# thu-ml/stochastic_gcn

Hardware: AMD Instinct MI355X
Metric: training edges/s (SpMM) (higher is better)
Workload: dtype f32

## Files before the change

### stochastic_gcn_amd/csrc/sgcn_csplan.cpp

```cpp
#include "sgcn_host.h"
#include "../../include/sgcn.h"

#include <algorithm>
#include <atomic>
#include <climits>
#include <cmath>
#include <cstdint>
#include <cstdio>
#include <cstdlib>
#include <cstring>
#include <functional>
#include <memory>
#include <new>
#include <numeric>
#include <queue>
#include <thread>
#include <vector>

#include <sched.h>

namespace {

struct VRow { int32_t row, piece, npieces, nnz; };

int plan_threads(int32_t requested) {
    if (requested > 0) return std::min<int32_t>(requested, 256);
    if (const char* e = getenv("SGCN_PLAN_THREADS")) {
        const int v = atoi(e);
        if (v > 0) return std::min(v, 256);
    }
    int n = (int)std::thread::hardware_concurrency();
    cpu_set_t set;
    if (sched_getaffinity(0, sizeof(set), &set) == 0) n = CPU_COUNT(&set);
    if (FILE* f = fopen("/sys/fs/cgroup/cpu.max", "r")) {
        char q[64] = {0};
        long long period = 0;
        if (fscanf(f, "%63s %lld", q, &period) == 2 && strcmp(q, "max") != 0 && period > 0) {
            const long long quota = atoll(q);
            if (quota > 0) n = (int)std::min<long long>(n, std::max<long long>(1, quota / period));
        }
        fclose(f);
    }
    return std::max(1, std::min(n, 64));
}

template <class F>
bool run_threads(int nthr, F fn) {
    std::atomic<int> bad{0};
    auto guarded = [&](int tid) {
        try { fn(tid); } catch (...) { bad.store(1); }
    };
    if (nthr <= 1) { guarded(0); return !bad.load(); }
    std::vector<std::thread> pool;
    pool.reserve((size_t)nthr - 1);
    try {
        for (int t = 1; t < nthr; t++) pool.emplace_back(guarded, t);
    } catch (...) { bad.store(1); }
    guarded(0);
    for (auto& th : pool) th.join();
    return !bad.load();
}

template <class F>
bool parallel_chunks(int64_t n, int64_t chunk, int nthr, F fn) {
    if (n <= 0) return true;
    chunk = std::max<int64_t>(1, chunk);
    nthr = (int)std::max<int64_t>(1, std::min<int64_t>(nthr, (n + chunk - 1) / chunk));
    std::atomic<int64_t> next{0};
    return run_threads(nthr, [&](int tid) {
        for (;;) {
            const int64_t b = next.fetch_add(chunk);
            if (b >= n) break;
            fn(b, std::min(n, b + chunk), tid);
        }
    });
}

void bucket_rows(const int32_t* row_group, int32_t M, std::vector<int32_t>& order, std::vector<int64_t>& gptr) {
    order.resize((size_t)M);
    if (!row_group) {
        std::iota(order.begin(), order.end(), 0);
        gptr = {0, (int64_t)M};
        return;
    }
    int32_t ng = 0;
    for (int32_t r = 0; r < M; r++) ng = std::max(ng, row_group[r] + 1);
    gptr.assign((size_t)ng + 1, 0);
    for (int32_t r = 0; r < M; r++) gptr[(size_t)row_group[r] + 1]++;
    for (int32_t g = 0; g < ng; g++) gptr[(size_t)g + 1] += gptr[g];
    std::vector<int64_t> fill(gptr.begin(), gptr.end() - 1);
    for (int32_t r = 0; r < M; r++) order[(size_t)fill[row_group[r]]++] = r;
}

inline int32_t default_t(const int32_t* rowptr, int32_t M) {
    const int64_t avg = M > 0 ? ((int64_t)rowptr[M] - rowptr[0]) / M : 0;
    return (int32_t)std::min<int64_t>(1024, std::max<int64_t>(64, 8 * avg));
}

void make_vrows(const int32_t* rowptr, const int32_t* rows, int64_t nrows, int32_t T, std::vector<VRow>& v) {
    std::vector<VRow> tmp;
    tmp.reserve((size_t)nrows + 64);
    int32_t wmax = 0;
    for (int64_t ri = 0; ri < nrows; ri++) {
        const int32_t r = rows[ri];
        const int32_t n = rowptr[r + 1] - rowptr[r];
        if (n <= T) { tmp.push_back({r, 0, 1, n}); wmax = std::max(wmax, n); continue; }
        const int32_t c = (n + T - 1) / T;
        for (int32_t q = 0; q < c; q++) {
            const int32_t w = (n - q + c - 1) / c;
            tmp.push_back({r, q, c, w});
            wmax = std::max(wmax, w);
        }
    }
    std::vector<int64_t> start((size_t)wmax + 2, 0);
    for (const VRow& x : tmp) start[(size_t)(wmax - x.nnz) + 1]++;
    for (size_t i = 1; i < start.size(); i++) start[i] += start[i - 1];
    const size_t base = v.size();
    v.resize(base + tmp.size());
    for (const VRow& x : tmp) v[base + (size_t)start[(size_t)(wmax - x.nnz)]++] = x;
}

void deal(const VRow* v, int64_t nv, int64_t vbase, int32_t R, int64_t nbins, int64_t* assign) {
    std::fill(assign, assign + nbins * R, (int64_t)-1);
    std::vector<int32_t> fill((size_t)nbins, 0);
    typedef std::pair<int64_t, int64_t> WT;
    std::priority_queue<WT, std::vector<WT>, std::greater<WT>> heap;
    for (int64_t t = 0; t < nbins; t++) heap.push({0, t});
    for (int64_t i = 0; i < nv; i++) {
        WT top = heap.top();
        heap.pop();
        const int64_t t = top.second;
        assign[t * R + fill[t]++] = vbase + i;
        if (fill[t] < R) heap.push({top.first + v[i].nnz, t});
    }
}

struct Layout {
    int32_t R = 16;
    int32_t NG = 1;
    std::vector<VRow> v;
    std::vector<int64_t> assign;
    int64_t ntiles = 0;
};

void layout_g1(const int32_t* rowptr, int32_t M, int32_t R, int32_t T, const int32_t* row_group, Layout& L) {
    std::vector<int32_t> order;
    std::vector<int64_t> gptr;
    bucket_rows(row_group, M, order, gptr);
    L.R = R; L.NG = 1; L.ntiles = 0;
    std::vector<int64_t> first_tile, vbase;
    for (size_t g = 0; g + 1 < gptr.size(); g++) {
        vbase.push_back((int64_t)L.v.size());
        make_vrows(rowptr, order.data() + gptr[g], gptr[g + 1] - gptr[g], T, L.v);
        first_tile.push_back(L.ntiles);
        L.ntiles += ((int64_t)L.v.size() - vbase.back() + R - 1) / R;
    }
    L.assign.resize((size_t)L.ntiles * R);
    for (size_t g = 0; g + 1 < gptr.size(); g++) {
        const int64_t nv = (g + 2 < gptr.size() ? vbase[g + 1] : (int64_t)L.v.size()) - vbase[g];
        const int64_t nt = (nv + R - 1) / R;
        deal(L.v.data() + vbase[g], nv, vbase[g], R, nt, L.assign.data() + first_tile[g] * R);
    }
}

constexpr int kG2R = 16;
void layout_gn(const int32_t* rowptr, int32_t M, int32_t T, int32_t round_tiles, int NG, Layout& L) {
    std::vector<int32_t> rows((size_t)M);
    std::iota(rows.begin(), rows.end(), 0);
    make_vrows(rowptr, rows.data(), M, T, L.v);
    const int64_t nv = (int64_t)L.v.size();
    int64_t nt = (nv + NG * kG2R - 1) / (NG * kG2R);
    if (round_tiles > 0 && nt > round_tiles / 2)
        nt = (nt + round_tiles - 1) / round_tiles * round_tiles;
    L.R = kG2R; L.NG = NG; L.ntiles = nt;
    L.assign.resize((size_t)nt * NG * kG2R);
    deal(L.v.data(), nv, 0, kG2R, nt * NG, L.assign.data());
}

struct Csr {
    const int32_t* rowptr = nullptr;
    const int32_t* col = nullptr;
    const float* val = nullptr;
    std::vector<int32_t> own_col;
    std::vector<float> own_val;
};

int prepare_csr(const int32_t* rowptr, const int32_t* col, const float* val, int32_t M, int bits, int nthr, Csr& A) {
    A.rowptr = rowptr; A.col = col; A.val = val;
    std::atomic<int> unsorted{0}, bad{0};
    const int64_t lim = (int64_t)1 << bits;
    if (!parallel_chunks(M, 2048, nthr, [&](int64_t r0, int64_t r1, int) {
            int u = 0, b = 0;
            for (int64_t r = r0; r < r1; r++)
                for (int32_t p = rowptr[r]; p < rowptr[r + 1]; p++) {
                    b |= (col[p] < 0) | ((int64_t)col[p] >= lim);
                    if (p > rowptr[r]) u |= col[p] < col[p - 1];
                }
            if (u) unsorted.store(1);
            if (b) bad.store(1);
        })) return 2;
    if (bad.load()) return 1;
    if (!unsorted.load()) return 0;
    const int64_t nnz = (int64_t)rowptr[M] - rowptr[0];
    const int64_t p0 = rowptr[0];
    try {
        A.own_col.resize((size_t)nnz);
        if (val) A.own_val.resize((size_t)nnz);
    } catch (...) { return 2; }
    if (!parallel_chunks(M, 512, nthr, [&](int64_t r0, int64_t r1, int) {
            std::vector<std::pair<int32_t, float>> buf;
            for (int64_t r = r0; r < r1; r++) {
                buf.clear();
                for (int32_t p = rowptr[r]; p < rowptr[r + 1]; p++) buf.push_back({col[p], val ? val[p] : 0.f});
                std::stable_sort(buf.begin(), buf.end(),
                                 [](const std::pair<int32_t, float>& a, const std::pair<int32_t, float>& b) { return a.first < b.first; });
                for (size_t i = 0; i < buf.size(); i++) {
                    A.own_col[(size_t)(rowptr[r] - p0) + i] = buf[i].first;
                    if (val) A.own_val[(size_t)(rowptr[r] - p0) + i] = buf[i].second;
                }
            }
        })) return 2;
    A.col = A.own_col.data() - p0;
    if (val) A.val = A.own_val.data() - p0;
    return 0;
}

struct Ent { uint32_t col, pos; float val; uint32_t lr; };
struct Scratch { std::vector<Ent> a, b; std::vector<uint32_t> runs, runs2; };

const std::vector<Ent>& gather_bin(const Layout& L, const Csr& A, int64_t bin, const uint32_t* warp, int32_t wshift, Scratch& S) {
    S.a.clear();
    S.runs.clear();
    S.runs.push_back(0);
    for (int32_t k = 0; k < L.R; k++) {
        const int64_t vi = L.assign[(size_t)bin * L.R + k];
        if (vi < 0) continue;
        const VRow& vr = L.v[(size_t)vi];
        const int32_t b = A.rowptr[vr.row], e = A.rowptr[vr.row + 1];
        for (int32_t p = b + vr.piece; p < e; p += vr.npieces) {
            const uint32_t c = (uint32_t)A.col[p];
            S.a.push_back({c, warp ? warp[c >> wshift] : c, A.val ? A.val[p] : 0.f, (uint32_t)k});
        }
        if (S.a.size() > S.runs.back()) S.runs.push_back((uint32_t)S.a.size());
    }
    std::vector<Ent>* src = &S.a;
    std::vector<Ent>* dst = &S.b;
    std::vector<uint32_t>* rs = &S.runs;
    std::vector<uint32_t>* rd = &S.runs2;
    while (rs->size() > 2) {
        dst->resize(src->size());
        rd->clear();
        rd->push_back(0);
        const size_t nr = rs->size() - 1;
        for (size_t i = 0; i < nr; i += 2) {
            const uint32_t lo = (*rs)[i], mid = (*rs)[i + 1], hi = i + 1 < nr ? (*rs)[i + 2] : mid;
            const Ent* x = src->data() + lo;
            const Ent* xe = src->data() + mid;
            const Ent* y = xe;
            const Ent* ye = src->data() + hi;
// ... 17 lines not shown
    int64_t step = 0;
    uint32_t window = 0;
    for (;;) {
        int64_t lo = INT64_MAX;
        uint32_t lo_col = 0;
        for (int g = 0; g < NG; g++)
            if (pos[g] < e[g]->size() && (int64_t)(*e[g])[pos[g]].pos < lo) { lo = (*e[g])[pos[g]].pos; lo_col = (*e[g])[pos[g]].col; }
        if (lo == INT64_MAX) break;
        window = lo_col;
        for (int g = 0; g < NG; g++) {
            const bool has = pos[g] < e[g]->size();
            const bool take = has && (align <= 0 || (int64_t)(*e[g])[pos[g]].pos <= lo + align);
            emit(g, take ? &(*e[g])[pos[g]] : nullptr, window);
            pos[g] += take;
        }
        step++;
    }
    const int64_t per_chunk = 64 / NG;
    while (step % per_chunk != 0) {
        for (int g = 0; g < NG; g++) emit(g, nullptr, window);
        step++;
    }
    return step;
}

inline uint64_t pack_entry(uint32_t word, float v) {
    uint32_t bits;
    memcpy(&bits, &v, 4);
    return (uint64_t)word | ((uint64_t)bits << 32);
}

}

struct sgcn_csbuild {
    int32_t G = 1, R = 16, T = 0;
    int64_t ntiles = 0, nentries = 0, nfix = 0, nslots = 0;
    bool count_only = false;
    std::vector<int64_t> tile_ptr;
    std::vector<int32_t> tile_rows, tile_slots;
    std::vector<sgcn_fix_t> fix;
    std::unique_ptr<uint64_t[]> flat;
    std::vector<std::vector<uint64_t>> arena;
    std::vector<int32_t> tile_tid;
    std::vector<int64_t> tile_off;
    int nthreads = 1;
};

namespace {

int build_plan(const int32_t* rowptr, const int32_t* col, const float* val, int32_t M, int32_t G, int32_t R, int32_t T,
               int32_t round_tiles, int32_t align, const int32_t* row_group, const uint32_t* warp, int32_t wshift,
               int32_t nthreads, bool count_only, sgcn_csbuild* B) {
    const int nthr = plan_threads(nthreads);
    B->G = G; B->R = G == 1 ? R : kG2R; B->nthreads = nthr; B->count_only = count_only;
    if (T <= 0) T = default_t(rowptr, M);
    B->T = T;
    if (row_group)
        for (int32_t r = 0; r < M; r++)
            if (row_group[r] < 0) return sgcn::fail(SGCN_ERR_INVALID, "csplan_build: negative group label at row %d", r);
    std::vector<int32_t> first_slot((size_t)M, -1);
    {
        int64_t slot = 0;
        for (int32_t r = 0; r < M; r++) {
            const int64_t n = (int64_t)rowptr[r + 1] - rowptr[r];
            if (n < 0) return sgcn::fail(SGCN_ERR_INVALID, "csplan_build: rowptr not monotone at %d", r);
            if (n <= T) continue;
            const int32_t c = (int32_t)((n + T - 1) / T);
            first_slot[r] = (int32_t)slot;
            B->fix.push_back(sgcn_fix_t{r, (int32_t)slot, c});
            slot += c;
            if (slot > INT32_MAX) return sgcn::fail(SGCN_ERR_INVALID, "csplan_build: too many workspace slots");
        }
        B->nfix = (int64_t)B->fix.size();
        B->nslots = slot;
    }
    const int bits = (G == 1 && R > 16) ? 27 : 28;
    Csr A;
    if (M > 0) {
        const int rc = prepare_csr(rowptr, col, val, M, bits, nthr, A);
        if (rc == 1) return sgcn::fail(SGCN_ERR_INVALID, "csplan_build: a column does not fit %d bits", bits);
        if (rc == 2) return sgcn::fail(SGCN_ERR_INVALID, "csplan_build: out of host memory");
    }
    Layout L;
    if (G == 1) layout_g1(rowptr, M, R, T, row_group, L);
    else layout_gn(rowptr, M, T, round_tiles, G, L);
    const int64_t nt = L.ntiles;
    const int32_t RR = L.R * L.NG;
    B->ntiles = nt;
    B->tile_ptr.assign((size_t)nt + 1, 0);
    B->tile_rows.resize((size_t)nt * RR);
    B->tile_slots.resize((size_t)nt * RR);
    auto fill_rows = [&](int64_t t) {
        for (int32_t k = 0; k < RR; k++) {
            const int64_t s = t * RR + k;
            const int64_t vi = L.assign[(size_t)s];
            if (vi < 0) { B->tile_rows[(size_t)s] = -1; B->tile_slots[(size_t)s] = -1; continue; }
            const VRow& vr = L.v[(size_t)vi];
            B->tile_rows[(size_t)s] = vr.row;
            B->tile_slots[(size_t)s] = vr.npieces > 1 ? first_slot[vr.row] + vr.piece : -1;
        }
    };
    const uint32_t shift = (uint32_t)bits;
    if (G == 1) {
        for (int64_t t = 0; t < nt; t++) {
            int64_t n = 0;
            for (int32_t k = 0; k < RR; k++) {
                const int64_t vi = L.assign[(size_t)(t * RR + k)];
                if (vi >= 0) n += L.v[(size_t)vi].nnz;
            }
            B->tile_ptr[(size_t)t + 1] = B->tile_ptr[(size_t)t] + n;
        }
        B->nentries = B->tile_ptr[(size_t)nt];
        if (count_only) { for (int64_t t = 0; t < nt; t++) fill_rows(t); return SGCN_OK; }
        B->flat.reset(new (std::nothrow) uint64_t[(size_t)std::max<int64_t>(B->nentries, 1)]);
        if (!B->flat) return sgcn::fail(SGCN_ERR_INVALID, "csplan_build: out of host memory");
        uint64_t* flat = B->flat.get();
        const bool ok = parallel_chunks(nt, 8, nthr, [&](int64_t t0, int64_t t1, int) {
            Scratch S;
            for (int64_t t = t0; t < t1; t++) {
                fill_rows(t);
                const std::vector<Ent>& e = gather_bin(L, A, t, nullptr, 0, S);
                uint64_t* o = flat + B->tile_ptr[(size_t)t];
                for (const Ent& en : e) *o++ = pack_entry(en.col | (en.lr << shift), en.val);
            }
        });
        if (!ok) return sgcn::fail(SGCN_ERR_INVALID, "csplan_build: out of host memory");
        return SGCN_OK;
    }
    B->arena.resize((size_t)nthr);
    B->tile_tid.assign((size_t)nt, 0);
    B->tile_off.assign((size_t)nt, 0);
    std::vector<int64_t> tile_len((size_t)nt, 0);
    const int64_t nnz = M > 0 ? (int64_t)rowptr[M] - rowptr[0] : 0;
    const int NG = G;
    const bool ok = parallel_chunks(nt, 8, nthr, [&](int64_t t0, int64_t t1, int tid) {
        Scratch S[4];
        const std::vector<Ent>* e[4] = {nullptr, nullptr, nullptr, nullptr};
        std::vector<uint64_t>& ar = B->arena[(size_t)tid];
        if (!count_only && ar.capacity() == 0) ar.reserve((size_t)(nnz / nthr + nnz / (4 * nthr) + 4096));
        for (int64_t t = t0; t < t1; t++) {
            fill_rows(t);
            for (int g = 0; g < NG; g++) e[g] = &gather_bin(L, A, NG * t + g, warp, wshift, S[g]);
            B->tile_tid[(size_t)t] = tid;
            B->tile_off[(size_t)t] = (int64_t)ar.size();
            int64_t steps;
            if (count_only) {
                steps = gn_schedule(e, NG, align, [](int, const Ent*, uint32_t) {});
            } else {
                steps = gn_schedule(e, NG, align, [&](int, const Ent* en, uint32_t window) {
                    if (en) {
                        float v = en->val;
                        uint32_t bts;
                        memcpy(&bts, &v, 4);
                        if (bts == kPadBits) v = 0.0f;
                        ar.push_back(pack_entry(en->col | (en->lr << 28), v));
                    } else {
                        ar.push_back((uint64_t)window | ((uint64_t)kPadBits << 32));
                    }
                });
            }
            tile_len[(size_t)t] = steps * NG;
        }
    });
    if (!ok) return sgcn::fail(SGCN_ERR_INVALID, "csplan_build: out of host memory");
    for (int64_t t = 0; t < nt; t++) B->tile_ptr[(size_t)t + 1] = B->tile_ptr[(size_t)t] + tile_len[(size_t)t];
    B->nentries = B->tile_ptr[(size_t)nt];
    return SGCN_OK;
}

int export_plan(const sgcn_csbuild* B, int64_t* tile_ptr, int32_t* colrow, float* valout, int32_t* tile_rows,
                int32_t* tile_slots, sgcn_fix_t* fix) {
    if (B->count_only) return sgcn::fail(SGCN_ERR_INVALID, "csbuild_export: a count-only build holds no entries");
    if (B->ntiles > 0 && (!tile_ptr || !tile_rows || !tile_slots)) return sgcn::fail(SGCN_ERR_INVALID, "csbuild_export: bad argument");
    if (B->nentries > 0 && (!colrow || !valout)) return sgcn::fail(SGCN_ERR_INVALID, "csbuild_export: bad argument");
    if (B->nfix > 0 && !fix) return sgcn::fail(SGCN_ERR_INVALID, "csbuild_export: split rows but no fix array");
    if (tile_ptr) memcpy(tile_ptr, B->tile_ptr.data(), B->tile_ptr.size() * sizeof(int64_t));
    if (B->tile_rows.size()) {
        memcpy(tile_rows, B->tile_rows.data(), B->tile_rows.size() * sizeof(int32_t));
        memcpy(tile_slots, B->tile_slots.data(), B->tile_slots.size() * sizeof(int32_t));
    }
    if (B->nfix) memcpy(fix, B->fix.data(), B->fix.size() * sizeof(sgcn_fix_t));
    auto split = [&](const uint64_t* src, int64_t n, int64_t at) {
        for (int64_t i = 0; i < n; i++) {
            colrow[at + i] = (int32_t)(uint32_t)src[i];
            const uint32_t bits = (uint32_t)(src[i] >> 32);
            memcpy(valout + at + i, &bits, 4);
        }
    };
    if (B->G == 1) {
        parallel_chunks(B->nentries, 1 << 18, B->nthreads, [&](int64_t b, int64_t e, int) { split(B->flat.get() + b, e - b, b); });
        return SGCN_OK;
    }
    parallel_chunks(B->ntiles, 8, B->nthreads, [&](int64_t t0, int64_t t1, int) {
        for (int64_t t = t0; t < t1; t++)
            split(B->arena[(size_t)B->tile_tid[(size_t)t]].data() + B->tile_off[(size_t)t],
                  B->tile_ptr[(size_t)t + 1] - B->tile_ptr[(size_t)t], B->tile_ptr[(size_t)t]);
    });
    return SGCN_OK;
}

}

extern "C" {

int sgcn_csplan_build(const int32_t* rowptr, const int32_t* col, const float* val, int32_t M, int32_t ngroups, int32_t R,
                      int32_t T, int32_t round_tiles, int32_t align, const int32_t* row_group, const uint32_t* host_warp,
                      int32_t warp_shift, int32_t nthreads, sgcn_csbuild_t** out) {
    if (!out) return sgcn::fail(SGCN_ERR_INVALID, "csplan_build: bad argument");
    *out = nullptr;
    if (M < 0 || (M > 0 && (!rowptr || !col || !val))) return sgcn::fail(SGCN_ERR_INVALID, "csplan_build: bad argument");
    if (ngroups != 1 && ngroups != 2 && ngroups != 4) return sgcn::fail(SGCN_ERR_INVALID, "csplan_build: one, two or four lane groups per wavefront");
    if (ngroups == 1 && (R < 1 || R > 32)) return sgcn::fail(SGCN_ERR_INVALID, "csplan_build: 1 <= R <= 32");
    if (ngroups != 1 && row_group) return sgcn::fail(SGCN_ERR_INVALID, "csplan_build: plans with lane groups are ungrouped");
    if (host_warp && (warp_shift < 0 || warp_shift > 27)) return sgcn::fail(SGCN_ERR_INVALID, "csplan_build: bad warp_shift");
    sgcn_csbuild* B = new (std::nothrow) sgcn_csbuild();
    if (!B) return sgcn::fail(SGCN_ERR_INVALID, "csplan_build: out of host memory");
    int rc;
    try {
        rc = build_plan(rowptr, col, val, M, ngroups, R, T, round_tiles, align, row_group, host_warp, warp_shift, nthreads, false, B);
    } catch (...) {
        rc = sgcn::fail(SGCN_ERR_INVALID, "csplan_build: out of host memory");
    }
    if (rc != SGCN_OK) { delete B; return rc; }
    *out = B;
    return SGCN_OK;
}

int sgcn_csbuild_sizes(const sgcn_csbuild_t* b, int64_t* ntiles, int64_t* nentries, int64_t* nfix, int64_t* nslots,
                       int32_t* T_used, int32_t* threads_used) {
    if (!b) return sgcn::fail(SGCN_ERR_INVALID, "csbuild_sizes: bad argument");
    if (ntiles) *ntiles = b->ntiles;
    if (nentries) *nentries = b->nentries;
    if (nfix) *nfix = b->nfix;
    if (nslots) *nslots = b->nslots;
    if (T_used) *T_used = b->T;
    if (threads_used) *threads_used = b->nthreads;
    return SGCN_OK;
}

int sgcn_csbuild_export(const sgcn_csbuild_t* b, int64_t* tile_ptr, int32_t* colrow, float* valout, int32_t* tile_rows,
                        int32_t* tile_slots, sgcn_fix_t* fix) {
    if (!b) return sgcn::fail(SGCN_ERR_INVALID, "csbuild_export: bad argument");
    return export_plan(b, tile_ptr, colrow, valout, tile_rows, tile_slots, fix);
}

void sgcn_csbuild_free(sgcn_csbuild_t* b) { delete b; }

// ... 244 lines not shown
```

### stochastic_gcn_amd/csrc/sgcn_spmm.hip

```cpp
#include "sgcn_dev.h"
#include <cstring>

namespace sgcn {

namespace {
int g_tune_nv = 0;
int g_tune_unroll = 0;
int g_tune_slabmajor = 1;
int g_tune_cs_round = 0;
int g_tune_cs_unroll = 0;
int g_tune_cs_pace = 0;
int g_tune_cs_slack = 0;
int g_tune_cs_noextra = 0;
int g_tune_step_overlap = 1;
int g_tune_step_fuse = 127;
int g_tune_cs_g2_wide = 0;
int g_tune_cs_nowarp = 0;
int g_tune_cs_last_pct = 80;
int g_tune_gemm_min_steps = 0;
int g_tune_gemm_mb16_slice_k = 0;
int g_tune_lds_wave_bias = 100;
int g_tune_lds_mix = 1;
int g_tune_lds_dbg = 0;
thread_local int tl_step_overlap = -1, tl_step_fuse = -1;
}

void step_mode_override(int overlap, int fuse) { tl_step_overlap = overlap; tl_step_fuse = fuse; }

int tune_get(const char* key) {
    if (!strcmp(key, "spmm_nv")) return g_tune_nv;
    if (!strcmp(key, "spmm_unroll")) return g_tune_unroll;
    if (!strcmp(key, "spmm_slabmajor")) return g_tune_slabmajor;
    if (!strcmp(key, "cs_round")) return g_tune_cs_round;
    if (!strcmp(key, "cs_unroll")) return g_tune_cs_unroll;
    if (!strcmp(key, "cs_pace")) return g_tune_cs_pace;
    if (!strcmp(key, "cs_slack")) return g_tune_cs_slack;
    if (!strcmp(key, "cs_noextra")) return g_tune_cs_noextra;
    if (!strcmp(key, "step_overlap")) return tl_step_overlap >= 0 ? tl_step_overlap : g_tune_step_overlap;
    if (!strcmp(key, "step_fuse")) return tl_step_fuse >= 0 ? tl_step_fuse : g_tune_step_fuse;
    if (!strcmp(key, "cs_g2_wide")) return g_tune_cs_g2_wide;
    if (!strcmp(key, "cs_nowarp")) return g_tune_cs_nowarp;
    if (!strcmp(key, "cs_last_pct")) return g_tune_cs_last_pct;
    if (!strcmp(key, "gemm_min_steps")) return g_tune_gemm_min_steps;
    if (!strcmp(key, "gemm_mb16_slice_k")) return g_tune_gemm_mb16_slice_k;
    if (!strcmp(key, "lds_wave_bias")) return g_tune_lds_wave_bias;
    if (!strcmp(key, "lds_mix")) return g_tune_lds_mix;
    if (!strcmp(key, "lds_dbg")) return g_tune_lds_dbg;
    return -1;
}

struct SpmmArgs {
    const int32_t* rowptr;
    const int32_t* col;
    const float* val;
    const sgcn_seg_t* seg;
    int64_t nseg;
    int64_t nsegblk;
    const void* B;
    int64_t ldb;
    const int32_t* gidx;
    const float* rscale;
    const float* cscale;
    float* C;
    int64_t ldc;
    float beta;
    int32_t d;
    int32_t nvec;
    float* ws;
    int64_t ldw;
    int32_t slabmajor;
    const float* add;
    int64_t ldadd;
    int32_t add_rows;
};

template <int VW>
__device__ __forceinline__ void epilogue_store(const SpmmArgs& a, int row, int vi,
                                               typename Vec<VW>::type acc, float rs) {
    float* out = a.C + (int64_t)row * a.ldc + (int64_t)vi * VW;
    typename Vec<VW>::type r = acc * rs;
    const int left = a.d - vi * VW;
    if (a.beta != 0.f) {
        if (left >= VW) r += a.beta * vload<VW>(out);
        else {
#pragma unroll
            for (int e = 0; e < VW; e++)
                if (e < left) {
                    if constexpr (VW == 1) r += a.beta * out[0]; else r[e] += a.beta * out[e];
                }
        }
    }
    if (a.add && row < a.add_rows) {
        const float* ad = a.add + (int64_t)row * a.ldadd + (int64_t)vi * VW;
        if (left >= VW) r += vload<VW>(ad);
        else {
#pragma unroll
            for (int e = 0; e < VW; e++)
                if (e < left) {
                    if constexpr (VW == 1) r += ad[0]; else r[e] += ad[e];
                }
        }
    }
    if (left >= VW) vstore<VW>(out, r);
    else vstore_head<VW>(out, r, left);
}

template <int G, int NV, int VW, int U, class BT>
__global__ __launch_bounds__(kBlock) void spmm_seg_kernel(SpmmArgs a) {
    typedef typename Vec<VW>::type VT;
    typedef typename HRaw<BT, VW>::type RT;
    constexpr bool kB16 = !std::is_same<BT, float>::value;
    constexpr int GPB = kBlock / G;
    const int lig = threadIdx.x & (G - 1);
    const int gib = threadIdx.x / G;

    int slab;
    int64_t sblk;
    if (a.slabmajor) { slab = (int)(blockIdx.x / a.nsegblk); sblk = blockIdx.x % a.nsegblk; }
    else { const int nslab = (int)(gridDim.x / a.nsegblk); slab = blockIdx.x % nslab; sblk = blockIdx.x / nslab; }
    const int64_t s = sblk * GPB + gib;
// ... 72 lines not shown
        for (int k = 0; k < NV; k++)
            if (act[k]) epilogue_store<VW>(a, row, vbase + k * G, acc[k], rs);
    } else {
        float* w = a.ws + (int64_t)slot * a.ldw + (int64_t)vbase * VW;
#pragma unroll
        for (int k = 0; k < NV; k++)
            if (act[k]) vstore<VW>(w + (int64_t)k * G * VW, acc[k]);
    }
}

template <int VW>
__global__ __launch_bounds__(kBlock) void spmm_fix_kernel(SpmmArgs a, const sgcn_fix_t* fix,
                                                          int64_t nfix) {
    typedef typename Vec<VW>::type VT;
    const int nvblk = (a.nvec + kBlock - 1) / kBlock;
    const int64_t f = blockIdx.x / nvblk;
    if (f >= nfix) return;
    const sgcn_fix_t fx = fix[f];
    const int vi = (int)(blockIdx.x % nvblk) * kBlock + threadIdx.x;
    if (vi >= a.nvec) return;
    const float* w = a.ws + (int64_t)fx.first_slot * a.ldw + (int64_t)vi * VW;
    VT acc = vzero<VW>();
    for (int q = 0; q < fx.nslots; q++) acc += vload<VW>(w + (int64_t)q * a.ldw);
    const float rs = a.rscale ? a.rscale[fx.row] : 1.0f;
    epilogue_store<VW>(a, fx.row, vi, acc, rs);
}

template <int G, int NV, int VW, int U, class BT>
static void launch_seg(const SpmmArgs& a, int64_t nblocks, hipStream_t st) {
    hipLaunchKernelGGL((spmm_seg_kernel<G, NV, VW, U, BT>), dim3((unsigned)nblocks), dim3(kBlock), 0, st, a);
}

template <int VW, int U, class BT>
static bool dispatch_gnv(int G, int NV, const SpmmArgs& a, int64_t nblocks, hipStream_t st) {
    switch (G) {
        case 8: launch_seg<8, 1, VW, U, BT>(a, nblocks, st); return true;
        case 16: launch_seg<16, 1, VW, U, BT>(a, nblocks, st); return true;
        case 32: launch_seg<32, 1, VW, U, BT>(a, nblocks, st); return true;
        case 64:
            switch (NV) {
                case 1: launch_seg<64, 1, VW, U, BT>(a, nblocks, st); return true;
                case 2: launch_seg<64, 2, VW, U, BT>(a, nblocks, st); return true;
                case 3: launch_seg<64, 3, VW, U, BT>(a, nblocks, st); return true;
                case 4: launch_seg<64, 4, VW, U, BT>(a, nblocks, st); return true;
            }
    }
    return false;
}

template <int VW, class BT>
static bool dispatch_u(int U, int G, int NV, const SpmmArgs& a, int64_t nblocks, hipStream_t st) {
    switch (U) {
        case 2: return dispatch_gnv<VW, 2, BT>(G, NV, a, nblocks, st);
        case 4: return dispatch_gnv<VW, 4, BT>(G, NV, a, nblocks, st);
        case 8: return dispatch_gnv<VW, 8, BT>(G, NV, a, nblocks, st);
    }
    return false;
}

int group_lanes(int nvec) {
    if (nvec <= 8) return 8;
    if (nvec <= 16) return 16;
    if (nvec <= 32) return 32;
    return 64;
}

}

using namespace sgcn;

extern "C" int64_t sgcn_tune_get(const char* key) { return key ? tune_get(key) : -1; }

extern "C" int sgcn_tune(const char* key, int64_t value) {
    if (!key) return fail(SGCN_ERR_INVALID, "sgcn_tune: null key");
    if (!strcmp(key, "spmm_nv")) { SGCN_REQUIRE(value >= 0 && value <= 4, "spmm_nv in 0..4"); g_tune_nv = (int)value; return SGCN_OK; }
    if (!strcmp(key, "spmm_unroll")) {
        SGCN_REQUIRE(value == 0 || value == 2 || value == 4 || value == 8, "spmm_unroll in {0,2,4,8}");
        g_tune_unroll = (int)value; return SGCN_OK;
    }
    if (!strcmp(key, "spmm_slabmajor")) { g_tune_slabmajor = value != 0; return SGCN_OK; }
    if (!strcmp(key, "cs_pace")) { SGCN_REQUIRE(value >= 0, "cs_pace >= 0"); g_tune_cs_pace = (int)value; return SGCN_OK; }
    if (!strcmp(key, "cs_slack")) { SGCN_REQUIRE(value >= 0, "cs_slack >= 0"); g_tune_cs_slack = (int)value; return SGCN_OK; }
    if (!strcmp(key, "cs_noextra")) { g_tune_cs_noextra = value != 0; return SGCN_OK; }
    if (!strcmp(key, "step_overlap")) { g_tune_step_overlap = value != 0; return SGCN_OK; }
    if (!strcmp(key, "step_fuse")) { SGCN_REQUIRE(value >= 0 && value <= 127, "step_fuse in 0..127"); g_tune_step_fuse = (int)value; return SGCN_OK; }
    if (!strcmp(key, "cs_g2_wide")) { g_tune_cs_g2_wide = value != 0; return SGCN_OK; }
    if (!strcmp(key, "cs_nowarp")) { g_tune_cs_nowarp = value != 0; return SGCN_OK; }
    if (!strcmp(key, "gemm_min_steps")) { g_tune_gemm_min_steps = (int)value; return SGCN_OK; }
    if (!strcmp(key, "gemm_mb16_slice_k")) {
        SGCN_REQUIRE(value >= 0 && value <= 0x7fffffff, "gemm_mb16_slice_k >= 0");
        g_tune_gemm_mb16_slice_k = (int)value; return SGCN_OK;
    }
    if (!strcmp(key, "lds_wave_bias")) { SGCN_REQUIRE(value >= 50 && value <= 300, "lds_wave_bias in 50..300 (per cent)"); g_tune_lds_wave_bias = (int)value; return SGCN_OK; }
    if (!strcmp(key, "lds_mix")) { g_tune_lds_mix = value != 0; return SGCN_OK; }
    if (!strcmp(key, "lds_dbg")) { g_tune_lds_dbg = (int)value; return SGCN_OK; }
    if (!strcmp(key, "cs_last_pct")) { SGCN_REQUIRE(value >= 0 && value <= 100, "cs_last_pct in [0, 100]"); g_tune_cs_last_pct = (int)value; return SGCN_OK; }
    if (!strcmp(key, "cs_round")) { SGCN_REQUIRE(value >= 0, "cs_round >= 0"); g_tune_cs_round = (int)value; return SGCN_OK; }
    if (!strcmp(key, "cs_unroll")) {
        SGCN_REQUIRE(value == 0 || value == 4 || value == 8, "cs_unroll in {0,4,8}");
        g_tune_cs_unroll = (int)value; return SGCN_OK;
    }
    return fail(SGCN_ERR_INVALID, "sgcn_tune: unknown key '%s'", key);
}

template <class BT>
static int spmm_csr_add(const int32_t* rowptr, const int32_t* col, const float* val,
                        int32_t M, int32_t K, int32_t d, const BT* B, int64_t ldb,
                        const int32_t* gidx, const float* rscale, const float* cscale,
                        float* C, int64_t ldc, float beta, const sgcn_plan_t* plan,
                        const float* add, int64_t ldadd, int32_t add_rows, void* stream) {
    constexpr bool kB16 = !std::is_same<BT, float>::value;
    SGCN_REQUIRE(M >= 0 && K >= 0 && d >= 0, "spmm: negative size");
    if (M == 0 || d == 0) return SGCN_OK;
    SGCN_REQUIRE(rowptr && C && (B || K == 0), "spmm: null operand");
    SGCN_REQUIRE(ldb >= d && ldc >= d, "spmm: leading dimension smaller than d");
    if (kB16) {
        SGCN_REQUIRE(ldb % 8 == 0, "spmm: a bfloat16 operand needs ldb %% 8 == 0 (ldb %lld, d %d)", (long long)ldb, d);
        SGCN_REQUIRE(aligned16(B), "spmm: a bfloat16 operand needs a 16-byte aligned base");
    }
    hipStream_t st = (hipStream_t)stream;

    SpmmArgs a{};
    a.rowptr = rowptr; a.col = col; a.val = val;
    a.B = B; a.ldb = ldb; a.gidx = gidx; a.rscale = rscale; a.cscale = cscale;
    a.C = C; a.ldc = ldc; a.beta = beta; a.d = d;
    a.nseg = M;
    a.slabmajor = g_tune_slabmajor;
    if (add && add_rows > 0) {
        SGCN_REQUIRE(ldadd >= d && add_rows <= M, "spmm: bad addend");
        a.add = add; a.ldadd = ldadd; a.add_rows = add_rows;
    }
    if (plan) {
        SGCN_REQUIRE(plan->dev_seg && plan->nseg >= M, "spmm: malformed plan");
        a.seg = plan->dev_seg; a.nseg = plan->nseg;
        a.ws = plan->dev_ws; a.ldw = ((int64_t)d + 3) / 4 * 4;
        if (plan->nfix > 0) {
            SGCN_REQUIRE(plan->dev_fix && plan->dev_ws, "spmm: plan with split rows needs dev_fix/dev_ws");
            SGCN_REQUIRE(plan->ws_elems >= plan->nslots * a.ldw,
                         "spmm: workspace too small (%lld < %lld floats)", (long long)plan->ws_elems,
                         (long long)(plan->nslots * a.ldw));
        }
    }
    const int vw = pick_vw(d, {kB16 ? nullptr : (const void*)B, C, plan ? plan->dev_ws : nullptr, a.add},
                           {ldb, ldc, a.add ? a.ldadd : ldc});
    a.nvec = (d + vw - 1) / vw;
    const int G = group_lanes(a.nvec);
    int NV = 1;
    if (G == 64) {
        const int per_wave = (a.nvec + 63) / 64;
        const int nslab0 = (per_wave + 3) / 4;
        NV = (per_wave + nslab0 - 1) / nslab0;
        if (g_tune_nv > 0) NV = g_tune_nv;
    }
    const int nslab = (a.nvec + G * NV - 1) / (G * NV);
    const int U = g_tune_unroll > 0 ? g_tune_unroll : (NV >= 3 ? 4 : 8);
    a.nsegblk = (a.nseg + (kBlock / G) - 1) / (kBlock / G);
    const int64_t nblocks = a.nsegblk * nslab;
    SGCN_REQUIRE(nblocks < (1ll << 31), "spmm: grid too large");

    bool ok = false;
    if (vw == 4) ok = dispatch_u<4, BT>(U, G, NV, a, nblocks, st);
    else if (vw == 2) ok = dispatch_u<2, BT>(U, G, NV, a, nblocks, st);
    else ok = dispatch_u<1, BT>(U, G, NV, a, nblocks, st);
    SGCN_REQUIRE(ok, "spmm: no kernel for G=%d NV=%d U=%d", G, NV, U);
    SGCN_HIP_TRY(hipGetLastError());

// ... 48 lines not shown
```

### stochastic_gcn_amd/ops.py

```python
import ctypes as C
import time

import numpy as np
import torch

from . import _ffi
from ._ffi import check, lib
from .scheduler import build_plan


_STREAM_CACHE = None


def _stream():
    if _STREAM_CACHE is not None:
        return _STREAM_CACHE
    return torch.cuda.current_stream().cuda_stream


def pin_stream():
    global _STREAM_CACHE
    _STREAM_CACHE = torch.cuda.current_stream().cuda_stream


# ... 867 lines not shown
        finally:
            lib.sgcn_csbuild_free(h)
        return tile_ptr, colrow, valout, tile_rows, tile_slots, fix, nt.value, nfix.value, nslots.value

    @staticmethod
    def matrix_key(a):
        import zlib
        a = a.tocsr()
        crc = 0
        for x in (a.indptr, a.indices, a.data):
            crc = zlib.crc32(np.ascontiguousarray(x).view(np.uint8), crc)
        return "%dx%d:%d:%08x" % (a.shape[0], a.shape[1], a.nnz, crc)

    @staticmethod
    def choose_g(d, avg_degree=None, rows=None):
        if avg_degree is not None and avg_degree <= 40 and rows is not None and rows > 4096 * 32:
            return 4
        dp = (int(d) + 3) // 4 * 4
        r1 = r2 = None
        if rows is not None and rows > 0:
            r1, r2 = -(-int(rows) // (4096 * 16)), -(-int(rows) // (4096 * 32))
        if r1 is None:
            r1, r2 = 2, 1
        return 2 if -(-dp // 128) * 0.73 * r2 <= -(-dp // 320) * r1 else 1

    def save(self, path, key):
        if self.grouped or self.ranged:
            raise ValueError("grouped / column-range plans are not cached (they are cheap to rebuild)")
        t = lambda x: x.cpu().numpy()
        blob = dict(key=np.array(key), G=self.G, pad_fraction=float(self.pad_fraction),
                    R=self.R, shape=np.array(self.shape, np.int64), nslots=self.nslots,
                    round_tiles=self.round_tiles, tile_ptr=t(self.tile_ptr), colrow=t(self.colrow), val=t(self.val),
                    tile_rows=t(self.tile_rows), tile_slots=t(self.tile_slots),
                    fix=t(self.fix) if self.fix is not None else np.zeros((0, 3), np.int32),
                    warp=t(self.warp) if self.warp is not None else np.zeros(0, np.int32), warp_shift=self.warp_shift)
        for clock, (pace_key, tuned_key) in zip(self._clocks, self.CLOCK_KEYS):
            blob[pace_key], blob[tuned_key] = clock.to_npz()
        import os
        import tempfile
        os.makedirs(os.path.dirname(path) or ".", exist_ok=True)
        fd, tmp = tempfile.mkstemp(prefix=os.path.basename(path) + ".", suffix=".tmp", dir=os.path.dirname(path) or ".")
        try:
            with os.fdopen(fd, "wb") as f:
                np.savez(f, **blob)
            os.replace(tmp, path)
        except BaseException:
            try:
                os.unlink(tmp)
            except OSError:
                pass
            raise

    @classmethod
    def load(cls, path, device, key, g=None):
        import os
        if not os.path.exists(path):
            return None
        try:
            return cls._load(path, device, key, g)
        except Exception:
            return None

    @classmethod
    def _load(cls, path, device, key, g):
        z = np.load(path)
        if str(z["key"]) != key:
            return None
        G = int(z["G"]) if "G" in z.files else 1
        if g is not None and G != g:
            return None
        warp = z["warp"] if "warp" in z.files and z["warp"].shape[0] else None
        p = dict(cls._RECORD, G=G, R=int(z["R"]), shape=tuple(int(x) for x in z["shape"]), nnz=int(z["colrow"].shape[0]),
                 pad_fraction=float(z["pad_fraction"]) if "pad_fraction" in z.files else 0.0, nslots=int(z["nslots"]),
                 warp=warp, warp_shift=int(z["warp_shift"]) if warp is not None else 0,
                 **{k: z[k] for k in ("tile_ptr", "colrow", "val", "tile_rows", "tile_slots", "fix")})
        self = cls.__new__(cls)
        self._finish(p, device, int(z["round_tiles"]), tuple(SweepClock.from_npz(z, *keys) for keys in cls.CLOCK_KEYS))
        return self

    @classmethod
    def cached(cls, a, device, path=None, G=1):
        if path is None:
            return cls(a, device, G=G), False
        key = "%s:r%d:Tauto:aauto:w1" % (cls.matrix_key(a), _cs_round())
        hit = cls.load(path, device, key, g=G)
        if hit is not None:
            return hit, True
        plan = cls(a, device, G=G)
        plan._cache = (path, key)
        return plan, False

    def store_if_cached(self):
        if self._cache is not None:
            try:
                self.save(*self._cache)
            except OSError:
                pass

    def struct(self, d, bf16=False):
        self.ws = _fixup_ws(self.ws, self.nslots, d, self.device)
        rnd = _cs_round(self.round_tiles)
        if self._hint_round != rnd:
            nl = -(-self.ntiles // rnd)
            pad = np.zeros(nl * rnd, dtype=np.int64)
            pad[:self.ntiles] = self._tile_nnz
            self._hint = np.ascontiguousarray(pad.reshape(nl, rnd).max(axis=1))
            self._hint_round = rnd
        return _ffi.CsPlan(self.R, self.ntiles, self.tile_ptr.data_ptr(), self.colrow.data_ptr(),
                           (self.val if self.live_val is None else self.live_val).data_ptr(), self.tile_rows.data_ptr(),
                           self.tile_slots.data_ptr(),
                           _ptr(self.fix), self.nfix, self.nslots, _ptr(self.ws),
                           0 if self.ws is None else self.ws.numel(), rnd, self._hint.ctypes.data,
                           -1 if self.grouped else int(self.clock(bf16).pace.get(d, 0)), self.G,
                           1 if (self.grouped or self.ranged) else 0, _ptr(self.warp), self.warp_shift)

    def variant(self, d, bf16=False):
        buf = C.create_string_buffer(256)
        plan = self.struct(d, bf16)
        check((lib.sgcn_spmm_cs_variant_b16 if bf16 else lib.sgcn_spmm_cs_variant)(C.byref(plan), int(d), buf, 256))
        return buf.value.decode()

    def autotune(self, B, d=None, candidates=None, reps=2, refine=True):
        d = int(B.shape[1] if d is None else d)
        self._tuning = True
        try:
            return self._autotune(B, d, candidates, reps, refine)
        finally:
            self._tuning = False

    def _autotune(self, B, d, candidates, reps, refine):
        if candidates is None:
            candidates = (-1, 230, 250, 270, 290, 310, 340, 380) if self.ranged else \
                (-1, 200, 220, 240, 260, 280, 320, 380) if self.G == 1 else \
                (-1, 130, 160, 190, 210, 230, 250, 280, 320)
        clock = self.clock(B.dtype == torch.bfloat16)
        pace_of, tuned_of, guard_of = clock.pace, clock.tuned_ms, clock.guard
        if self.grouped:
            pace_of[d] = -1
            return (None, -1)
        out = _pitched_out(self.shape[0], d, B.device)
        def timed(p, reps=reps):
            pace_of[d] = p
            spmm_cs(self, B, out=out, d=d)
            e0, e1 = torch.cuda.Event(enable_timing=True), torch.cuda.Event(enable_timing=True)
            e0.record()
            for _ in range(reps):
                spmm_cs(self, B, out=out, d=d)
            e1.record()
            e1.synchronize()
            return e0.elapsed_time(e1) / reps

        best = None
        for p in candidates:
            t = timed(p)
            if best is None or t < best[0]:
                best = (t, p)
        ext = 0
        while refine and best[1] > 0 and best[1] == max(candidates) and best[1] < 2000 and ext < 8:
            ext += 1
            p = max(best[1] + 1, int(best[1] * 1.15))
            candidates = tuple(candidates) + (p,)
            t = timed(p)
            if t < best[0]:
                best = (t, p)
        if refine and best[1] > 0:
            for p in sorted({int(best[1] * f) for f in (0.94, 0.96, 0.98, 1.02)} - set(candidates)):
                t = timed(p)
# ... 684 lines not shown
```

Measured before the change: 7.656 billion.

## Deal rows to bins by column-distribution balance and sort tiles by length

Adds a column-aware dealing step for G>1 column-sweep plans. Each row's columns are histogrammed into 64 buckets, and the row goes to whichever near-lightest bin keeps its cumulative column profile closest to the sweep clock. After dealing, tiles are reordered longest-first, so each round is led by its heaviest tiles. The aim is to cut padding and the skew between bins and tiles in the lock-step sweep, at the cost of a more expensive host-side plan build. The new path is on by default through a new cs_deal knob, and the plan cache key now includes that knob.

```diff
diff --git a/profiles/cs_deal_probe.py b/profiles/cs_deal_probe.py
--- /dev/null
+++ b/profiles/cs_deal_probe.py
@@ -0,0 +1,215 @@
+#!/usr/bin/env python
+import argparse
+import csv
+import glob
+import json
+import os
+import sys
+import time
+
+import numpy as np
+
+ROOT = os.path.dirname(os.path.dirname(os.path.abspath(__file__)))
+sys.path.insert(0, ROOT)
+
+D = 602
+PAD = 0x80000000
+
+
+def _matrix(small=False):
+    from stochastic_gcn_amd import synthetic
+    if small:
+        return synthetic.reddit_like(n=23296, m=1160000, splits=(15241, 2369, 5533), seed=1, with_features=False)[2].tocsr()
+    return synthetic.reddit_like(with_features=False)[2].tocsr()
+
+
+def _deal(v):
+    from stochastic_gcn_amd._ffi import check, lib
+    check(lib.sgcn_tune(b"cs_deal", int(v)))
+
+
+def plan_stats(tile_ptr, colrow, val, G, rnd, K, nnz):
+    tp = np.asarray(tile_ptr, np.int64)
+    nt = tp.shape[0] - 1
+    steps = np.diff(tp) // G
+    nl = -(-nt // rnd)
+    padded = np.zeros(nl * rnd, np.int64)
+    padded[:nt] = steps
+    per_round = padded.reshape(nl, rnd)
+    real = np.asarray(val).view(np.uint32) != PAD
+    tile = np.repeat(np.arange(nt), np.diff(tp))
+    e = np.arange(tp[-1]) - tp[tile]
+    bin_id = tile * G + e % G
+    clock = (e // G) * (K / np.maximum(per_round.max(axis=1), 1)[tile // rnd])
+    col = (np.asarray(colrow).view(np.uint32) & 0x0FFFFFFF).astype(np.float64)
+    off = np.zeros(nt * G)
+    np.maximum.at(off, bin_id[real], np.abs(col - clock)[real])
+    live = np.bincount(bin_id[real], minlength=nt * G)
+    return {"ntiles": int(nt), "rounds": int(nl), "pad_fraction": round(1.0 - nnz / max(int(tp[-1]), 1), 4),
+            "heaviest_tile_steps_per_round": per_round.max(axis=1).tolist(),
+            "mean_tile_steps": round(float(steps[steps > 0].mean()), 1), "ideal_steps": round(nnz / max(int((live > 0).sum()), 1), 1),
+            "bin_off_clock_columns_mean_p90": [round(float(off[live > 0].mean())), round(float(np.percentile(off[live > 0], 90)))],
+            "heaviest_bin_nnz": int(live.max()), "mean_bin_nnz": round(float(live[live > 0].mean()), 1)}
+
+
+def cpu(args):
+    from stochastic_gcn_amd import ops
+    Cs = ops.ColumnSweepCSR
+    a = _matrix(args.small)
+    for name, m in (("A", a), ("A^T", ops.transpose_host(a))):
+        m = m.tocsr()
+        rowptr, col = np.ascontiguousarray(m.indptr, np.int32), np.ascontiguousarray(m.indices, np.int32)
+        val = np.ascontiguousarray(m.data, np.float32)
+        M, K = m.shape
+        G = args.cs_g
+        rnd = args.round or ops._cs_round(None)
+        T = Cs.auto_t(rowptr, G, rnd)
+        wtab, shift = Cs.make_warp(col, K, 'auto')
+        align = args.align or Cs.auto_align(K, col.shape[0], M, G, rnd)
+        for deal in [int(x) for x in args.deals.split(',')]:
+            _deal(deal)
+            secs = {}
+            for label, threads in (("all_threads", args.threads), ("one_thread", 1)):
+                t0 = time.perf_counter()
+                built = Cs._build(rowptr, col, val, M, G, 16, T, rnd, int(align), None,
+                                  wtab.ctypes.data if wtab is not None else None, shift, threads=threads)
+                secs[label] = round(time.perf_counter() - t0, 3)
+            rec = {"what": "plan", "matrix": name, "graph": "sreddit-small" if args.small else "sreddit", "cs_deal": deal, "G": G,
+                   "round": rnd, "align": int(align), "T": int(T), "warp": wtab is not None, "build_s": secs}
+            rec.update(plan_stats(built[0], built[1], built[2], G, rnd, K, m.nnz))
+            print(json.dumps(rec), flush=True)
+        if args.small or not args.transpose:
+            break
+
+
+def _setup(deals, bf16=False):
+    import torch
+    from stochastic_gcn_amd import ops
+    from profiles.spmm_b16_probe import _guard_off, _operands
+    dev = torch.device("cuda:0")
+    a = _matrix()
+    n = a.shape[0]
+    at = ops.transpose_host(a)
+    G = ops.ColumnSweepCSR.choose_g(D, a.nnz / max(n, 1), n)
+    plans, build_s = {}, {}
+    for deal in deals:
+        _deal(deal)
+        t0 = time.perf_counter()
+        plans[deal] = (ops.ColumnSweepCSR(a, dev, G=G), ops.ColumnSweepCSR(at, dev, G=G))
+        build_s[deal] = round(time.perf_counter() - t0, 3)
+        _guard_off(*plans[deal])
+    X, dC = _operands(n, D, dev, bf16)
+    out = torch.empty((n, (D + 3) // 4 * 4), device=dev)[:, :D]
+    out_t = torch.empty((n, (D + 3) // 4 * 4), device=dev)[:, :D]
+    return plans, build_s, X, dC, out, out_t, G
+
+
+def _describe(A, AT):
+    A.struct(D), AT.struct(D)
+    return {"kernel": A.variant(D), "pad_fraction": [round(float(A.pad_fraction), 4), round(float(AT.pad_fraction), 4)],
+            "heaviest_tile_steps_per_launch": [A._hint.tolist(), AT._hint.tolist()], "nfix": [A.nfix, AT.nfix]}
+
+
+def products(args):
+    from stochastic_gcn_amd import ops
+    from profiles.spmm_b16_probe import _sustained
+    plans, build_s, X, dC, out, out_t, G = _setup((0, 1), args.bf16)
+
+    def pair(deal):
+        A, AT = plans[deal]
+        return lambda: (ops.spmm_cs(A, X, out=out), ops.spmm_cs(AT, dC, out=out_t))
+
+    tuned = {}
+    for deal, (A, AT) in plans.items():
+        bf, bb = A.autotune(X), AT.autotune(dC)
+        tuned[deal] = dict(fwd_ms=bf[0], fwd_pace=bf[1], bwd_ms=bb[0], bwd_pace=bb[1])
+        for P in (A, AT):
+            P._guard.clear()
+    runs = {deal: [] for deal in plans}
+    for _ in range(args.repeats):
+        for deal in plans:
+            runs[deal].append(_sustained(pair(deal), args.iters))
+    for deal, (A, AT) in plans.items():
+        ms = runs[deal]
+        rec = {"what": "products", "cs_deal": deal, "operand": "bf16" if args.bf16 else "fp32", "graph": "sreddit", "d": D, "G": G, "tuned": tuned[deal], "iters": args.iters,
+               "repeats": args.repeats, "pair_ms": ms, "pair_ms_mean": sum(ms) / len(ms), "pair_ms_min": min(ms),
+               "pair_ms_max": max(ms), "plans_build_and_upload_s": build_s[deal]}
+        rec.update(_describe(A, AT))
+        print(json.dumps(rec), flush=True)
+    o, t = runs[0], runs[1]
+    width = max(o) - min(o)
+    print(json.dumps({"what": "products verdict", "deal1_minus_deal0_ms": sum(t) / len(t) - sum(o) / len(o),
+                      "deal0_min_max": [min(o), max(o)], "deal1_min_max": [min(t), max(t)],
+                      "gap_over_deal0_range_width": (min(o) - max(t)) / width if width > 0 else None,
+                      "note": "recorded, not a gate"}), flush=True)
+
+
+def paces(args):
+    from stochastic_gcn_amd import ops
+    from profiles.spmm_b16_probe import _sustained
+    plans, _, X, dC, out, out_t, G = _setup((0, 1))
+    for p in [int(x) for x in args.paces.split(",")]:
+        ms = {}
+        for deal, (A, AT) in plans.items():
+            A.pace[D] = AT.pace[D] = p
+            ms[deal] = []
+        for _ in range(args.repeats):
+            for deal, (A, AT) in plans.items():
+                ms[deal].append(_sustained(lambda: (ops.spmm_cs(A, X, out=out), ops.spmm_cs(AT, dC, out=out_t)), args.iters))
+        print(json.dumps({"what": "paces", "pace": p, "G": G, "iters": args.iters, "pair_ms_by_cs_deal": ms}), flush=True)
+
+
+def run(args):
+    import torch
+    from stochastic_gcn_amd import ops
+    plans, _, X, dC, out, out_t, G = _setup((args.deal,))
+    A, AT = plans[args.deal]
+    A.pace[D], AT.pace[D] = args.pace_fwd, args.pace_bwd
+    for _ in range(args.iters):
+        ops.spmm_cs(A, X, out=out)
+        ops.spmm_cs(AT, dC, out=out_t)
+    torch.cuda.synchronize()
+    rec = {"what": "run", "cs_deal": args.deal, "iters": args.iters, "G": G, "pace_fwd": args.pace_fwd, "pace_bwd": args.pace_bwd}
+    rec.update(_describe(A, AT))
+    print(json.dumps(rec), flush=True)
+
+
+def kernels(args):
+    f = glob.glob(os.path.join(args.dir, "**", "*kernel_trace.csv"), recursive=True)
+    rows = list(csv.DictReader(open(f[0])))
+    for tag, key in (("sweep", "cs_spmm16"), ("fixup", "cs_fix_kernel")):
+        us = sorted((int(r["End_Timestamp"]) - int(r["Start_Timestamp"])) / 1e3 for r in rows if key in r["Kernel_Name"])
+        if us:
+            print(json.dumps({"what": "kernel", "dir": args.dir, "kernel": tag, "launches": len(us), "avg_us": sum(us) / len(us),
+                              "median_us": us[len(us) // 2], "min_us": us[0], "max_us": us[-1]}), flush=True)
+
+
+def main():
+    ap = argparse.ArgumentParser()
+    ap.add_argument("what", nargs="?", default=None, choices=["products", "paces", "run", "kernels"])
+    ap.add_argument("--cpu", action="store_true", help="plan statistics only (no GPU)")
+    ap.add_argument("--small", action="store_true", help="--cpu: the tests' small S-Reddit (round 256, align 224)")
+    ap.add_argument("--transpose", action="store_true", help="--cpu: the transposed matrix too")
+    ap.add_argument("--cs-g", type=int, default=2, choices=[2, 4])
+    ap.add_argument("--round", type=int, default=0)
+    ap.add_argument("--align", type=int, default=0)
+    ap.add_argument("--threads", type=int, default=0)
+    ap.add_argument("--deal", type=int, default=1)
+    ap.add_argument("--deals", default="0,1", help="--cpu: the knob values to build with")
+    ap.add_argument("--bf16", action="store_true", help="products: bfloat16 operands (the plans' bfloat16 clocks)")
+    ap.add_argument("--repeats", type=int, default=4)
+    ap.add_argument("--iters", type=int, default=40)
+    ap.add_argument("--pace-fwd", type=int, default=-1)
+    ap.add_argument("--pace-bwd", type=int, default=-1)
+    ap.add_argument("--paces", default="186,188,190,192,194,196,198,202")
+    ap.add_argument("--dir", default=None)
+    args = ap.parse_args()
+    if args.cpu:
+        return cpu(args)
+    if args.what is None:
+        ap.error("one of --cpu, products, paces, run, kernels")
+    {"products": products, "paces": paces, "run": run, "kernels": kernels}[args.what](args)
+
+
+if __name__ == "__main__":
+    main()
diff --git a/stochastic_gcn_amd/csrc/sgcn_csplan.cpp b/stochastic_gcn_amd/csrc/sgcn_csplan.cpp
--- a/stochastic_gcn_amd/csrc/sgcn_csplan.cpp
+++ b/stochastic_gcn_amd/csrc/sgcn_csplan.cpp
@@ -14,6 +14,7 @@
 #include <new>
 #include <numeric>
 #include <queue>
+#include <set>
 #include <thread>
 #include <vector>
 
@@ -135,6 +136,52 @@
     }
 }
 
+constexpr int kDealBuckets = 64, kDealCand = 32;
+
+struct DealCols {
+    const int32_t* rowptr;
+    const int32_t* col;
+    const uint32_t* warp;
+    int32_t wshift;
+    uint64_t scale;
+    inline int bucket(int64_t p) const {
+        const uint32_t c = (uint32_t)col[p];
+        return (int)(((uint64_t)(warp ? warp[c >> wshift] : c) * scale) >> 32);
+    }
+};
+
+void deal_aware(const VRow* v, int64_t nv, int32_t R, int64_t nbins, const DealCols& A, int64_t* assign) {
+    constexpr int NB = kDealBuckets;
+    std::fill(assign, assign + nbins * R, (int64_t)-1);
+    std::vector<int64_t> off((size_t)nbins * NB, 0), w((size_t)nbins, 0);
+    std::vector<int32_t> fill((size_t)nbins, 0);
+    std::set<std::pair<int64_t, int64_t>> open;
+    for (int64_t t = 0; t < nbins; t++) open.insert(open.end(), {0, t});
+    int64_t h[NB];
+    for (int64_t i = 0; i < nv; i++) {
+        const VRow& x = v[i];
+        std::fill(h, h + NB, 0);
+        for (int64_t p = (int64_t)A.rowptr[x.row] + x.piece; p < A.rowptr[x.row + 1]; p += x.npieces) h[A.bucket(p)]++;
+        for (int64_t k = 0, cum = 0; k < NB; k++) { cum += h[k]; h[k] = cum * NB - (int64_t)x.nnz * (k + 1); }
+        const int64_t wmin = open.begin()->first, tol = std::max<int64_t>(8, x.nnz / 2);
+        int64_t best = -1, best_dev = INT64_MAX;
+        int seen = 0;
+        for (auto it = open.begin(); it != open.end() && seen < kDealCand && it->first <= wmin + tol; ++it, ++seen) {
+            const int64_t* ob = off.data() + (size_t)it->second * NB;
+            int64_t dev = 0;
+            for (int k0 = 0; k0 < 8 && dev < best_dev; k0++)
+                for (int k = 7 - k0; k < NB; k += 8) dev = std::max<int64_t>(dev, std::llabs(ob[k] + h[k]));
+            if (dev < best_dev) { best_dev = dev; best = it->second; }
+        }
+        open.erase({w[(size_t)best], best});
+        assign[best * R + fill[(size_t)best]++] = i;
+        int64_t* ob = off.data() + (size_t)best * NB;
+        for (int k = 0; k < NB; k++) ob[k] += h[k];
+        w[(size_t)best] += x.nnz;
+        if (fill[(size_t)best] < R) open.insert({w[(size_t)best], best});
+    }
+}
+
 struct Layout {
     int32_t R = 16;
     int32_t NG = 1;
@@ -164,7 +211,7 @@
 }
 
 constexpr int kG2R = 16;
-void layout_gn(const int32_t* rowptr, int32_t M, int32_t T, int32_t round_tiles, int NG, Layout& L) {
+void layout_gn(const int32_t* rowptr, int32_t M, int32_t T, int32_t round_tiles, int NG, const DealCols* cols, Layout& L) {
     std::vector<int32_t> rows((size_t)M);
     std::iota(rows.begin(), rows.end(), 0);
     make_vrows(rowptr, rows.data(), M, T, L.v);
@@ -174,7 +221,8 @@
         nt = (nt + round_tiles - 1) / round_tiles * round_tiles;
     L.R = kG2R; L.NG = NG; L.ntiles = nt;
     L.assign.resize((size_t)nt * NG * kG2R);
-    deal(L.v.data(), nv, 0, kG2R, nt * NG, L.assign.data());
+    if (!cols) { deal(L.v.data(), nv, 0, kG2R, nt * NG, L.assign.data()); return; }
+    deal_aware(L.v.data(), nv, kG2R, nt * NG, *cols, L.assign.data());
 }
 
 struct Csr {
@@ -358,8 +406,23 @@
         if (rc == 2) return sgcn::fail(SGCN_ERR_INVALID, "csplan_build: out of host memory");
     }
     Layout L;
+    const bool aware = G != 1 && M > 0 && sgcn_tune_get("cs_deal") > 0;
     if (G == 1) layout_g1(rowptr, M, R, T, row_group, L);
-    else layout_gn(rowptr, M, T, round_tiles, G, L);
+    else if (!aware) layout_gn(rowptr, M, T, round_tiles, G, nullptr, L);
+    else {
+        DealCols dc{A.rowptr, A.col, warp, wshift, 0};
+        std::vector<int64_t> top((size_t)nthr, 0);
+        if (!parallel_chunks((int64_t)rowptr[M] - rowptr[0], 1 << 18, nthr, [&](int64_t b, int64_t e, int tid) {
+                int64_t m = top[(size_t)tid];
+                for (int64_t p = rowptr[0] + b; p < rowptr[0] + e; p++) {
+                    const uint32_t c = (uint32_t)A.col[p];
+                    m = std::max<int64_t>(m, warp ? warp[c >> wshift] : c);
+                }
+                top[(size_t)tid] = m;
+            })) return sgcn::fail(SGCN_ERR_INVALID, "csplan_build: out of host memory");
+        dc.scale = ((uint64_t)kDealBuckets << 32) / (uint64_t)(*std::max_element(top.begin(), top.end()) + 1);
+        layout_gn(rowptr, M, T, round_tiles, G, &dc, L);
+    }
     const int64_t nt = L.ntiles;
     const int32_t RR = L.R * L.NG;
     B->ntiles = nt;
@@ -439,6 +502,19 @@
         }
     });
     if (!ok) return sgcn::fail(SGCN_ERR_INVALID, "csplan_build: out of host memory");
+    if (aware && round_tiles > 0 && nt > round_tiles) {
+        std::vector<int64_t> perm((size_t)nt);
+        std::iota(perm.begin(), perm.end(), 0);
+        std::stable_sort(perm.begin(), perm.end(), [&](int64_t a, int64_t b) { return tile_len[(size_t)a] > tile_len[(size_t)b]; });
+        std::vector<int64_t> len(tile_len), off(B->tile_off);
+        std::vector<int32_t> tid(B->tile_tid), rws(B->tile_rows), sls(B->tile_slots);
+        for (int64_t t = 0; t < nt; t++) {
+            const size_t s = (size_t)perm[(size_t)t];
+            tile_len[(size_t)t] = len[s]; B->tile_off[(size_t)t] = off[s]; B->tile_tid[(size_t)t] = tid[s];
+            std::copy(rws.begin() + s * RR, rws.begin() + (s + 1) * RR, B->tile_rows.begin() + t * RR);
+            std::copy(sls.begin() + s * RR, sls.begin() + (s + 1) * RR, B->tile_slots.begin() + t * RR);
+        }
+    }
     for (int64_t t = 0; t < nt; t++) B->tile_ptr[(size_t)t + 1] = B->tile_ptr[(size_t)t] + tile_len[(size_t)t];
     B->nentries = B->tile_ptr[(size_t)nt];
     return SGCN_OK;
diff --git a/stochastic_gcn_amd/csrc/sgcn_spmm.hip b/stochastic_gcn_amd/csrc/sgcn_spmm.hip
--- a/stochastic_gcn_amd/csrc/sgcn_spmm.hip
+++ b/stochastic_gcn_amd/csrc/sgcn_spmm.hip
@@ -12,6 +12,7 @@
 int g_tune_cs_pace = 0;
 int g_tune_cs_slack = 0;
 int g_tune_cs_noextra = 0;
+int g_tune_cs_deal = 1;
 int g_tune_step_overlap = 1;
 int g_tune_step_fuse = 127;
 int g_tune_cs_g2_wide = 0;
@@ -36,6 +37,7 @@
     if (!strcmp(key, "cs_pace")) return g_tune_cs_pace;
     if (!strcmp(key, "cs_slack")) return g_tune_cs_slack;
     if (!strcmp(key, "cs_noextra")) return g_tune_cs_noextra;
+    if (!strcmp(key, "cs_deal")) return g_tune_cs_deal;
     if (!strcmp(key, "step_overlap")) return tl_step_overlap >= 0 ? tl_step_overlap : g_tune_step_overlap;
     if (!strcmp(key, "step_fuse")) return tl_step_fuse >= 0 ? tl_step_fuse : g_tune_step_fuse;
     if (!strcmp(key, "cs_g2_wide")) return g_tune_cs_g2_wide;
@@ -274,6 +276,7 @@
     if (!strcmp(key, "cs_pace")) { SGCN_REQUIRE(value >= 0, "cs_pace >= 0"); g_tune_cs_pace = (int)value; return SGCN_OK; }
     if (!strcmp(key, "cs_slack")) { SGCN_REQUIRE(value >= 0, "cs_slack >= 0"); g_tune_cs_slack = (int)value; return SGCN_OK; }
     if (!strcmp(key, "cs_noextra")) { g_tune_cs_noextra = value != 0; return SGCN_OK; }
+    if (!strcmp(key, "cs_deal")) { SGCN_REQUIRE(value == 0 || value == 1, "cs_deal in {0, 1}"); g_tune_cs_deal = (int)value; return SGCN_OK; }
     if (!strcmp(key, "step_overlap")) { g_tune_step_overlap = value != 0; return SGCN_OK; }
     if (!strcmp(key, "step_fuse")) { SGCN_REQUIRE(value >= 0 && value <= 127, "step_fuse in 0..127"); g_tune_step_fuse = (int)value; return SGCN_OK; }
     if (!strcmp(key, "cs_g2_wide")) { g_tune_cs_g2_wide = value != 0; return SGCN_OK; }
diff --git a/stochastic_gcn_amd/ops.py b/stochastic_gcn_amd/ops.py
--- a/stochastic_gcn_amd/ops.py
+++ b/stochastic_gcn_amd/ops.py
@@ -973,7 +973,7 @@
     def cached(cls, a, device, path=None, G=1):
         if path is None:
             return cls(a, device, G=G), False
-        key = "%s:r%d:Tauto:aauto:w1" % (cls.matrix_key(a), _cs_round())
+        key = "%s:r%d:Tauto:aauto:w1:d%d" % (cls.matrix_key(a), _cs_round(), _ffi.lib.sgcn_tune_get(b"cs_deal"))
         hit = cls.load(path, device, key, g=G)
         if hit is not None:
             return hit, True
```

Result: faster. 7.786 billion (median of 6 runs) (+1.7%).
